# waiwnf/pilotguru

Measured on AMD Instinct MI355X. Metric: frames/sec ORB extract+match, 1080p @ 2000 kp/frame, higher is better.
Workload: dtype u8

## Files before the change

pilotguru_amd/csrc/describe.hip:

```cpp
#include "pgorb_internal.h"

struct PgGauss7 { int k0, k1, k2, k3; };
constexpr PgGauss7 PG_G7 = {18, 34, 49, 55};

#define DH_N 37

struct PgDescTab { uint32_t mom[5 * 64]; uint32_t btab[3 * 64 * 4]; int8_t pat[64 * 4 * 4]; };
constexpr PgDescTab pg_make_desc_tab()
{
    constexpr int umax[16] = {15, 15, 15, 15, 14, 14, 14, 13, 13, 12, 11, 10, 9, 8, 6, 3};
    constexpr int8_t p[256 * 4] = {
#include "orb_pattern31.inc"
    };
    constexpr int K[7] = {PG_G7.k0, PG_G7.k1, PG_G7.k2, PG_G7.k3, PG_G7.k2, PG_G7.k1, PG_G7.k0};
    PgDescTab t = {};
    for (int r = 0; r < 31; r++)
        for (int q = 0; q < 9; q++) {
            const int vy = r - 15, dmax = umax[vy < 0 ? -vy : vy];
            uint32_t wu = 0;
            for (int k = 0; k < 4; k++) {
                const int ux = 4 * (q + 1) + k - 21;
                if ((ux < 0 ? -ux : ux) <= dmax) wu |= (uint32_t)(ux + 16) << (8 * k);
            }
            t.mom[r * 9 + q] = wu;
        }
    for (int cb = 0; cb < 3; cb++)
        for (int l = 0; l < 64; l++)
            for (int j = 0; j < 16; j++) {
                const int k = 16 * (l >> 4) + j, n = 16 * cb + (l & 15), d = k - n;
                const uint32_t v = (d >= 0 && d <= 6 && n < DH_N) ? (uint32_t)K[d] : 0u;
                t.btab[(cb * 64 + l) * 4 + j / 4] |= v << (8 * (j % 4));
            }
    for (int l = 0; l < 64; l++)
        for (int r = 0; r < 4; r++)
            for (int k = 0; k < 4; k++) t.pat[(l * 4 + r) * 4 + k] = p[(64 * r + l) * 4 + k];
    return t;
}
__device__ static const __attribute__((aligned(16))) PgDescTab pg_desc_tab = pg_make_desc_tab();

#define DW_R 21
#define DW_N 43
#define DW_PITCH 48
#define DH_PITCH 40
#define DB_PITCH 40

__device__ __forceinline__ int pg_reflect101(int p, int n)
{
    if (n == 1) return 0;
    while (p < 0 || p >= n) p = (p < 0) ? -p : 2 * (n - 1) - p;
    return p;
}

__device__ __forceinline__ float pg_fast_atan2(float y, float x)
{
    const float scale = (float)(180 / 3.1415926535897932384626433832795);
    const float p1 = 0.9997878412794807f * scale, p3 = -0.3258083974640975f * scale;
    const float p5 = 0.1555786518463281f * scale, p7 = -0.04432655554792128f * scale;
    const float eps = (float)2.2204460492503131e-16;
    const float ax = fabsf(x), ay = fabsf(y);
    float a, c, c2;
    if (ax >= ay) {
        c = __fdiv_rn(ay, __fadd_rn(ax, eps));
        c2 = __fmul_rn(c, c);
        a = __fmul_rn(__fadd_rn(__fmul_rn(__fadd_rn(__fmul_rn(__fadd_rn(__fmul_rn(p7, c2), p5), c2), p3), c2), p1), c);
    } else {
        c = __fdiv_rn(ax, __fadd_rn(ay, eps));
        c2 = __fmul_rn(c, c);
        a = __fsub_rn(90.f, __fmul_rn(__fadd_rn(__fmul_rn(__fadd_rn(__fmul_rn(__fadd_rn(__fmul_rn(p7, c2), p5), c2), p3), c2), p1), c));
    }
    if (x < 0) a = __fsub_rn(180.f, a);
    if (y < 0) a = __fsub_rn(360.f, a);
    return a;
}

__device__ __forceinline__ void pg_sincos_f(float angle, float* s_out, float* c_out)
{
    const double INV_PIO2 = 0.63661977236758138243;
    const double PIO2_HI = 1.57079632673412561417e+00;
    const double PIO2_LO = 6.07710050650619224932e-11;
    const double x = (double)angle;
    const double kd = floor(__dadd_rn(__dmul_rn(x, INV_PIO2), 0.5));
    const double r = __dsub_rn(__dsub_rn(x, __dmul_rn(kd, PIO2_HI)), __dmul_rn(kd, PIO2_LO));
    const double r2 = __dmul_rn(r, r);
    double ps = -1.0 / 355687428096000.0;
    ps = __dadd_rn(__dmul_rn(ps, r2), 1.0 / 1307674368000.0);
    ps = __dsub_rn(__dmul_rn(ps, r2), 1.0 / 6227020800.0);
    ps = __dadd_rn(__dmul_rn(ps, r2), 1.0 / 39916800.0);
    ps = __dsub_rn(__dmul_rn(ps, r2), 1.0 / 362880.0);
    ps = __dadd_rn(__dmul_rn(ps, r2), 1.0 / 5040.0);
    ps = __dsub_rn(__dmul_rn(ps, r2), 1.0 / 120.0);
    ps = __dadd_rn(__dmul_rn(ps, r2), 1.0 / 6.0);
    const double sn = __dsub_rn(r, __dmul_rn(__dmul_rn(r, r2), ps));
    double pc = -1.0 / 6402373705728000.0;
    pc = __dadd_rn(__dmul_rn(pc, r2), 1.0 / 20922789888000.0);
    pc = __dsub_rn(__dmul_rn(pc, r2), 1.0 / 87178291200.0);
    pc = __dadd_rn(__dmul_rn(pc, r2), 1.0 / 479001600.0);
    pc = __dsub_rn(__dmul_rn(pc, r2), 1.0 / 3628800.0);
    pc = __dadd_rn(__dmul_rn(pc, r2), 1.0 / 40320.0);
    pc = __dsub_rn(__dmul_rn(pc, r2), 1.0 / 720.0);
    pc = __dadd_rn(__dmul_rn(pc, r2), 1.0 / 24.0);
    pc = __dsub_rn(__dmul_rn(pc, r2), 0.5);
    const double cs = __dadd_rn(1.0, __dmul_rn(r2, pc));
    const int k = (int)((long long)kd & 3);
    const double s = (k == 0) ? sn : (k == 1) ? cs : (k == 2) ? -sn : -cs;
    const double c = (k == 0) ? cs : (k == 1) ? -sn : (k == 2) ? -cs : sn;
    *s_out = (float)s;
    *c_out = (float)c;
}

__device__ __forceinline__ int pg_wave_sum(int x)
{
    int v = x;
    v += __builtin_amdgcn_update_dpp(0, v, 0x111, 0xf, 0xf, true);
    v += __builtin_amdgcn_update_dpp(0, v, 0x112, 0xf, 0xf, true);
    v += __builtin_amdgcn_update_dpp(0, v, 0x114, 0xf, 0xf, true);
    v += __builtin_amdgcn_update_dpp(0, v, 0x118, 0xf, 0xf, true);
    v += __builtin_amdgcn_update_dpp(0, v, 0x142, 0xa, 0xf, false);
    v += __builtin_amdgcn_update_dpp(0, v, 0x143, 0xc, 0xf, false);
    return __builtin_amdgcn_readlane(v, 63);
}


typedef __attribute__((address_space(1))) const void* pg_gptr_t;
typedef __attribute__((address_space(3))) void* pg_lptr_t;
typedef unsigned short pg_us2 __attribute__((ext_vector_type(2)));
typedef int pg_v4i __attribute__((ext_vector_type(4)));
#define PG_GLOBAL __attribute__((address_space(1)))
typedef PG_GLOBAL const uint8_t* pg_gbytes_t;

__device__ __forceinline__ int pg_blur_at(const uint32_t* hT, int Y, int X, bool tieEven)
{
    constexpr PgGauss7 G = PG_G7;
    const pg_us2 K01 = {(unsigned short)G.k0, (unsigned short)G.k1}, K23 = {(unsigned short)G.k2, (unsigned short)G.k3},
                 K45 = {(unsigned short)G.k2, (unsigned short)G.k1};
    const uint32_t* s = hT + (Y >> 1) * 40 + X;
    const uint32_t p0 = s[0], p1 = s[40], p2 = s[80], p3 = s[120];
    const uint32_t sh = (uint32_t)(Y & 1) << 4;
    const uint32_t a0 = __builtin_amdgcn_alignbit(p1, p0, sh), a1 = __builtin_amdgcn_alignbit(p2, p1, sh),
                   a2 = __builtin_amdgcn_alignbit(p3, p2, sh), last = (p3 >> sh) & 0xFFFFu;
    uint32_t C = __builtin_amdgcn_udot2(__builtin_bit_cast(pg_us2, a0), K01, (uint32_t)G.k0 * last, false);
    C = __builtin_amdgcn_udot2(__builtin_bit_cast(pg_us2, a1), K23, C, false);
    C = __builtin_amdgcn_udot2(__builtin_bit_cast(pg_us2, a2), K45, C, false);
    int v = (int)((C + 32768u) >> 16);
    if (tieEven && (C & 0xFFFFu) == 0x8000u) v &= ~1;
    return min(v, 255);
}

#define PG_WAVE_SYNC() do { __builtin_amdgcn_fence(__ATOMIC_RELEASE, "wavefront"); __builtin_amdgcn_wave_barrier(); \
                            __builtin_amdgcn_fence(__ATOMIC_ACQUIRE, "wavefront"); } while (0)

struct PgDescArgs {
    const int32_t* kpCount;  const PgSelRec* sel;  int64_t selFrame;  pgorb_keypoint* kps;
    uint8_t* desc;  int32_t* n_out;  int32_t nlevels, tieMode, cap_per_frame, slotBeg;
    int32_t slotEnd, writeTotal, slotsPerXcd, pad[5];
};
static_assert(sizeof(PgDescArgs) == 96 && sizeof(PgDescArgs) <= 128, "one s_load_dwordx16 + one s_load_dwordx8");

__global__ __launch_bounds__(64) void k_describe(const PgDescArgs KA)
{
    __shared__ __attribute__((aligned(16))) uint32_t hbuf[22 * DH_PITCH];
    uint8_t* raw = reinterpret_cast<uint8_t*>(hbuf);

    const int lane = threadIdx.x;
    const uint32_t frame = blockIdx.y;
    typedef int32_t pg_i32x16 __attribute__((ext_vector_type(16)));
    typedef uint32_t pg_u32x16 __attribute__((ext_vector_type(16)));
    typedef uint32_t pg_u32x8 __attribute__((ext_vector_type(8)));
    pg_gbytes_t tb = (pg_gbytes_t)(const void*)&pg_desc_tab;
    asm volatile("" : "+s"(tb));
    const uint32_t o4 = 4u * (uint32_t)lane, o16 = 16u * (uint32_t)lane;
    uint32_t mt[5];
#pragma unroll
    for (int it = 0; it < 5; it++) mt[it] = *(const PG_GLOBAL uint32_t*)(tb + (offsetof(PgDescTab, mom) + 256 * it) + o4);
    pg_v4i Bop[3];
#pragma unroll
    for (int cb = 0; cb < 3; cb++) Bop[cb] = *(const PG_GLOBAL pg_v4i*)(tb + (offsetof(PgDescTab, btab) + 1024 * cb) + o16);
    const pg_v4i pat = *(const PG_GLOBAL pg_v4i*)(tb + offsetof(PgDescTab, pat) + o16);
    pg_u32x16 a0;
    pg_u32x8 a1;
    asm volatile("s_load_dwordx16 %0, %2, 0x0\n\ts_load_dwordx8 %1, %2, 0x40\n\ts_waitcnt lgkmcnt(0)"
                 : "=&s"(a0), "=&s"(a1) : "s"(__builtin_amdgcn_kernarg_segment_ptr()) : "memory");
#define PG_A64(T, v, k) reinterpret_cast<T>((uintptr_t)(((uint64_t)(v)[(k) + 1] << 32) | (v)[k]))
    const int32_t* kpCount = PG_A64(const int32_t*, a0, 0);
    const PgSelRec* sel = PG_A64(const PgSelRec*, a0, 2);
    const int64_t selFrame = (int64_t)(((uint64_t)a0[5] << 32) | a0[4]);
    pgorb_keypoint* kps = PG_A64(pgorb_keypoint*, a0, 6);
    uint8_t* desc = PG_A64(uint8_t*, a0, 8);
    int32_t* n_out = PG_A64(int32_t*, a0, 10);
#undef PG_A64
    const int nlevels = (int)a0[12], tieMode = (int)a0[13], cap_per_frame = (int)a0[14], slotBeg = (int)a0[15];
    const int slotEnd = (int)a1[0], writeTotal = (int)a1[1], slotsPerXcd = (int)a1[2];
    const int slot = slotBeg + (int)(blockIdx.x & 7) * slotsPerXcd + (int)(blockIdx.x >> 3);
    const int32_t* kpc = kpCount + frame * PG_MAXL;
    const PgSelRec* recp = sel + ((int64_t)frame * selFrame + slot);
    pg_i32x16 kc;
    pg_u32x8 rec;
    asm volatile("s_load_dwordx16 %0, %2, 0x0\n\ts_load_dwordx8 %1, %3, 0x0\n\ts_waitcnt lgkmcnt(0)" : "=&s"(kc), "=&s"(rec) : "s"(kpc), "s"(recp) : "memory");
    if (slot >= slotEnd) return;
    const int l = (int)(rec[1] >> 16) & 15;
    int total = 0, before = 0;
#pragma unroll
    for (int q = 0; q < PG_MAXL; q++) {
        const int c = kc[q];
        if (q < l) before += c;
        total += c;
    }
    if (writeTotal && blockIdx.x == 0 && lane == 0) n_out[frame] = total;
    if (rec[1] == 0xFFFFFFFFu || l >= nlevels) return;
    const uint32_t cv = rec[0];
    const int idx = before + (int)(rec[1] & 0xFFFFu);
    const int Lpitch = (int)rec[2], Lw = (int)(rec[3] & 0xFFFFu), Lh = (int)(rec[3] >> 16);
    const uint8_t* img = reinterpret_cast<const uint8_t*>((uintptr_t)(((uint64_t)rec[5] << 32) | rec[4]));
    const float Lscale = __uint_as_float(rec[6]), LpatchSize = __uint_as_float(rec[7]);
    const int x = (int)(cv & 0xFFF) + PG_EDGE, y = (int)((cv >> 12) & 0xFFF) + PG_EDGE;
    const int resp = (int)(cv >> 24);
    const int w = Lw, h = Lh;

    const int x0 = x - DW_R, y0 = y - DW_R;
    if (x0 >= 0 && y0 >= 0 && x0 + DW_PITCH <= w && y + DW_R < h) {
        const int lr = lane / 3, lq = lane - 3 * lr;
        const uint8_t* g = img + (int64_t)(y0 + lr) * Lpitch + x0 + 16 * lq;
        if (lr < 21) {
            __builtin_amdgcn_global_load_lds((pg_gptr_t)g, (pg_lptr_t)raw, 16, 0, 0);
            __builtin_amdgcn_global_load_lds((pg_gptr_t)(g + 21 * (int64_t)Lpitch), (pg_lptr_t)(raw + 21 * DW_PITCH), 16, 0, 0);
            if (lr < 1)
                __builtin_amdgcn_global_load_lds((pg_gptr_t)(g + 42 * (int64_t)Lpitch), (pg_lptr_t)(raw + 42 * DW_PITCH), 16, 0, 0);
        }
        __builtin_amdgcn_s_waitcnt(0);
    } else {
        for (int i = lane; i < DW_N * DW_PITCH; i += 64) {
            const int r = i / DW_PITCH, c = i - r * DW_PITCH;
            raw[r * DW_PITCH + c] =
                img[(int64_t)pg_reflect101(y0 + r, h) * Lpitch + pg_reflect101(x0 + c, w)];
        }
    }
    PG_WAVE_SYNC();

    int m10 = 0, m01 = 0;
#pragma unroll
    for (int it = 0; it < 5; it++) {
        const int i = lane + 64 * it;
        if (i >= 31 * 9) break;
        const int r = i / 9, q = i - r * 9;
        const uint32_t val = *reinterpret_cast<const uint32_t*>(raw + (DW_R - 15 + r) * DW_PITCH + 4 * (q + 1));
        const uint32_t wm = ((mt[it] + 0x7F7F7F7Fu) >> 7) & 0x01010101u;
        const int sv = (int)__builtin_amdgcn_udot4(val, wm, 0u, false);
        m10 += (int)__builtin_amdgcn_udot4(val, mt[it], 0u, false) - 16 * sv;
        m01 += (r - 15) * sv;
    }
    m10 = pg_wave_sum(m10);
    m01 = pg_wave_sum(m01);
    const float angle = pg_fast_atan2((float)m01, (float)m10);

    uint32_t* hT = hbuf;
    {
        constexpr int cinit = 128 * (2 * (PG_G7.k0 + PG_G7.k1 + PG_G7.k2) + PG_G7.k3);
        pg_v4i Aop[3];
#pragma unroll
        for (int rb = 0; rb < 3; rb++) {
            Aop[rb] = *reinterpret_cast<const pg_v4i*>(raw + (16 * rb + (lane & 15)) * DW_PITCH + 16 * (lane >> 4));
            Aop[rb].x ^= (int)0x80808080; Aop[rb].y ^= (int)0x80808080; Aop[rb].z ^= (int)0x80808080; Aop[rb].w ^= (int)0x80808080;
        }
        PG_WAVE_SYNC();
#pragma unroll
        for (int rb = 0; rb < 3; rb++) {
            const int pair = 8 * rb + 2 * (lane >> 4);
#pragma unroll
            for (int cb = 0; cb < 3; cb++) {
                const pg_v4i acc = __builtin_amdgcn_mfma_i32_16x16x64_i8(Aop[rb], Bop[cb], pg_v4i{cinit, cinit, cinit, cinit}, 0, 0, 0);
                const int n = 16 * cb + (lane & 15);
                if (n < DH_PITCH) {
                    if (pair < 22) hT[pair * DH_PITCH + n] = (uint32_t)acc.x | ((uint32_t)acc.y << 16);
                    if (pair + 1 < 22) hT[(pair + 1) * DH_PITCH + n] = (uint32_t)acc.z | ((uint32_t)acc.w << 16);
                }
            }
        }
    }
    PG_WAVE_SYNC();
    const int wvec = w & ~3;

    const float factorPI = (float)(3.1415926535897932384626433832795 / 180.f);
    float a, b;
    pg_sincos_f(__fmul_rn(angle, factorPI), &b, &a);
    unsigned long long bits[4];
#pragma unroll
    for (int r = 0; r < 4; r++) {
        const uint32_t pw = (uint32_t)pat[r];
        const float px0 = (float)(int8_t)(pw & 0xFF), py0 = (float)(int8_t)((pw >> 8) & 0xFF);
        const float px1 = (float)(int8_t)((pw >> 16) & 0xFF), py1 = (float)(int8_t)(pw >> 24);
        const int r0 = __float2int_rn(__fadd_rn(__fmul_rn(px0, b), __fmul_rn(py0, a)));
        const int c0 = __float2int_rn(__fsub_rn(__fmul_rn(px0, a), __fmul_rn(py0, b)));
        const int r1 = __float2int_rn(__fadd_rn(__fmul_rn(px1, b), __fmul_rn(py1, a)));
        const int c1 = __float2int_rn(__fsub_rn(__fmul_rn(px1, a), __fmul_rn(py1, b)));
        const int t0 = pg_blur_at(hT, 18 + r0, 18 + c0, tieMode == 0 && x + c0 < wvec);
        const int t1 = pg_blur_at(hT, 18 + r1, 18 + c1, tieMode == 0 && x + c1 < wvec);
        bits[r] = __ballot(t0 < t1);
    }

    if (idx < cap_per_frame && lane == 0) {
        const int64_t o = (int64_t)frame * cap_per_frame + idx;
        unsigned long long* d = reinterpret_cast<unsigned long long*>(desc + o * 32);
        d[0] = bits[0]; d[1] = bits[1]; d[2] = bits[2]; d[3] = bits[3];
        pgorb_keypoint k;
        k.x = (l != 0) ? __fmul_rn((float)x, Lscale) : (float)x;
        k.y = (l != 0) ? __fmul_rn((float)y, Lscale) : (float)y;
        k.size = LpatchSize;
        k.angle = angle;
        k.response = (float)resp;
        k.octave = l;
        k.class_id = -1;
        kps[o] = k;
    }
}

static PgGauss7 pg_gauss7()
{
    float cf[7];
    double sum = 0;
    for (int i = 0; i < 7; i++) {
        const double xx = i - 3.0;
        cf[i] = (float)exp(-0.5 / (2.0 * 2.0) * xx * xx);
        sum += cf[i];
    }
    sum = 1. / sum;
    int K[7];
    for (int i = 0; i < 7; i++) {
        cf[i] = (float)(cf[i] * sum);
        K[i] = (int)lrint((double)(cf[i] * 256.f));
    }
    PgGauss7 g = {K[0], K[1], K[2], K[3]};
    return g;
}

bool pg_launch_describe(const PgPlan& P, int nframes, pgorb_keypoint* d_kps, uint8_t* d_desc,
                        int cap_per_frame, int32_t* d_n, hipStream_t s)
{
    return pg_launch_describe_levels(P, nframes, d_kps, d_desc, cap_per_frame, d_n, 0, P.nlevels, s);
}

bool pg_launch_describe_levels(const PgPlan& P, int nframes, pgorb_keypoint* d_kps, uint8_t* d_desc,
                               int cap_per_frame, int32_t* d_n, int levelBeg, int levelEnd, hipStream_t s)
{
    static const PgGauss7 G = pg_gauss7();
    static const bool tapsOk = G.k0 == PG_G7.k0 && G.k1 == PG_G7.k1 && G.k2 == PG_G7.k2 && G.k3 == PG_G7.k3;
    if (!tapsOk) return false;
    PgDescArgs KA = {};
    KA.kpCount = P.kpCount; KA.sel = reinterpret_cast<const PgSelRec*>(P.sel); KA.selFrame = P.selFrame;
    KA.kps = d_kps; KA.desc = d_desc; KA.n_out = d_n;
    KA.nlevels = P.nlevels; KA.tieMode = P.tieMode; KA.cap_per_frame = cap_per_frame;
    KA.slotBeg = (int)P.lvl[levelBeg].selOff;
    KA.slotEnd = (levelEnd < P.nlevels) ? (int)P.lvl[levelEnd].selOff : P.selTotal;
    KA.writeTotal = levelEnd == P.nlevels ? 1 : 0;
    dim3 grid((KA.slotEnd - KA.slotBeg + 7) & ~7, nframes), block(64);
    KA.slotsPerXcd = (int)(grid.x >> 3);
    hipLaunchKernelGGL(k_describe, grid, block, 0, s, KA);
    return true;
}

__global__ __launch_bounds__(256) void k_sincos_checksum(uint32_t first_bits, uint32_t count, unsigned long long* out)
{
    const uint32_t base = first_bits + blockIdx.x * count;
    unsigned long long acc = 0;
    for (uint32_t i = threadIdx.x; i < count; i += 256) {
        float s, c;
        pg_sincos_f(__uint_as_float(base + i), &s, &c);
        acc += ((unsigned long long)__float_as_uint(s) * 0x9E3779B1ull + __float_as_uint(c)) * (2ull * i + 1ull);
    }
    __shared__ unsigned long long red[256];
    red[threadIdx.x] = acc;
    __syncthreads();
    for (int st = 128; st > 0; st >>= 1) {
        if ((int)threadIdx.x < st) red[threadIdx.x] += red[threadIdx.x + st];
        __syncthreads();
    }
    if (threadIdx.x == 0) out[blockIdx.x] = red[0];
}

extern "C" int pgorb_debug_sincos_checksum(uint32_t first_bits, uint32_t count, int nblocks, unsigned long long* out)
{
    if (!out || nblocks < 1 || count < 1) return PGORB_E_ARG;
    unsigned long long* d = nullptr;
    if (hipMalloc((void**)&d, sizeof(unsigned long long) * (size_t)nblocks) != hipSuccess) return PGORB_E_HIP;
    hipLaunchKernelGGL(k_sincos_checksum, dim3(nblocks), dim3(256), 0, 0, first_bits, count, d);
    const bool ok = hipMemcpy(out, d, sizeof(unsigned long long) * (size_t)nblocks, hipMemcpyDeviceToHost) == hipSuccess;
    (void)hipFree(d);
    return ok ? 0 : PGORB_E_HIP;
}
```

Before: 99640.

## Restructure describe kernel moments, blur buffer layout, and tap address arithmetic

The moment table is reordered so each lane handles one column position across five rows spaced seven apart. This lets the per-row sums chain through udot4 accumulators and removes the per-iteration division and modulo. The blurred-row buffer pitch grows to 48 with 24 row pairs, so all nine MFMA results are stored without bounds checks, and the MFMAs are issued back to back before any stores. Sample coordinates are rounded with a float magic-number add, and the LDS address and tie-break comparison are computed directly from the float bits, replacing float-to-int conversions and integer index math. The larger buffer uses more LDS, and the bit tricks depend on coordinates staying inside a small range.

Result: no change. 100,200, median of 6 (+0.5%).

```diff
diff --git a/pilotguru_amd/csrc/describe.hip b/pilotguru_amd/csrc/describe.hip
--- a/pilotguru_amd/csrc/describe.hip
+++ b/pilotguru_amd/csrc/describe.hip
@@ -22,7 +22,7 @@
                 const int ux = 4 * (q + 1) + k - 21;
                 if ((ux < 0 ? -ux : ux) <= dmax) wu |= (uint32_t)(ux + 16) << (8 * k);
             }
-            t.mom[r * 9 + q] = wu;
+            t.mom[(r / 7) * 64 + (r % 7) * 9 + q] = wu;
         }
     for (int cb = 0; cb < 3; cb++)
         for (int l = 0; l < 64; l++)
@@ -41,7 +41,8 @@
 #define DW_R 21
 #define DW_N 43
 #define DW_PITCH 48
-#define DH_PITCH 40
+#define DH_PITCH 48
+#define DH_PAIRS 24
 #define DB_PITCH 40
 
 __device__ __forceinline__ int pg_reflect101(int p, int n)
@@ -128,14 +129,14 @@
 #define PG_GLOBAL __attribute__((address_space(1)))
 typedef PG_GLOBAL const uint8_t* pg_gbytes_t;
 
-__device__ __forceinline__ int pg_blur_at(const uint32_t* hT, int Y, int X, bool tieEven)
+typedef __attribute__((address_space(3))) const uint32_t* pg_lds_u32p;
+__device__ __forceinline__ int pg_blur_at(pg_lds_u32p s, uint32_t odd, bool tieEven)
 {
     constexpr PgGauss7 G = PG_G7;
     const pg_us2 K01 = {(unsigned short)G.k0, (unsigned short)G.k1}, K23 = {(unsigned short)G.k2, (unsigned short)G.k3},
                  K45 = {(unsigned short)G.k2, (unsigned short)G.k1};
-    const uint32_t* s = hT + (Y >> 1) * 40 + X;
-    const uint32_t p0 = s[0], p1 = s[40], p2 = s[80], p3 = s[120];
-    const uint32_t sh = (uint32_t)(Y & 1) << 4;
+    const uint32_t p0 = s[0], p1 = s[DH_PITCH], p2 = s[2 * DH_PITCH], p3 = s[3 * DH_PITCH];
+    const uint32_t sh = odd << 4;
     const uint32_t a0 = __builtin_amdgcn_alignbit(p1, p0, sh), a1 = __builtin_amdgcn_alignbit(p2, p1, sh),
                    a2 = __builtin_amdgcn_alignbit(p3, p2, sh), last = (p3 >> sh) & 0xFFFFu;
     uint32_t C = __builtin_amdgcn_udot2(__builtin_bit_cast(pg_us2, a0), K01, (uint32_t)G.k0 * last, false);
@@ -158,7 +159,7 @@
 
 __global__ __launch_bounds__(64) void k_describe(const PgDescArgs KA)
 {
-    __shared__ __attribute__((aligned(16))) uint32_t hbuf[22 * DH_PITCH];
+    __shared__ __attribute__((aligned(16))) uint32_t hbuf[DH_PAIRS * DH_PITCH];
     uint8_t* raw = reinterpret_cast<uint8_t*>(hbuf);
 
     const int lane = threadIdx.x;
@@ -236,17 +237,21 @@
     }
     PG_WAVE_SYNC();
 
-    int m10 = 0, m01 = 0;
-#pragma unroll
-    for (int it = 0; it < 5; it++) {
-        const int i = lane + 64 * it;
-        if (i >= 31 * 9) break;
-        const int r = i / 9, q = i - r * 9;
-        const uint32_t val = *reinterpret_cast<const uint32_t*>(raw + (DW_R - 15 + r) * DW_PITCH + 4 * (q + 1));
-        const uint32_t wm = ((mt[it] + 0x7F7F7F7Fu) >> 7) & 0x01010101u;
-        const int sv = (int)__builtin_amdgcn_udot4(val, wm, 0u, false);
-        m10 += (int)__builtin_amdgcn_udot4(val, mt[it], 0u, false) - 16 * sv;
-        m01 += (r - 15) * sv;
+    int m10, m01;
+    {
+        const int r0 = lane / 9, q = lane - 9 * r0;
+        const uint8_t* mrow = raw + (DW_R - 15 + r0) * DW_PITCH + 4 * (q + 1);
+        uint32_t val[5], S[5], mu = 0;
+#pragma unroll
+        for (int it = 0; it < 5; it++) val[it] = *reinterpret_cast<const uint32_t*>(mrow + 7 * it * DW_PITCH);
+#pragma unroll
+        for (int it = 0; it < 5; it++) {
+            const uint32_t wm = ((mt[it] + 0x7F7F7F7Fu) >> 7) & 0x01010101u;
+            S[it] = __builtin_amdgcn_udot4(val[it], wm, it ? S[it - 1] : 0u, false);
+            mu = __builtin_amdgcn_udot4(val[it], mt[it], mu, false);
+        }
+        m10 = (int)mu - 16 * (int)S[4];
+        m01 = __mul24(r0 + 13, (int)S[4]) - __mul24(7, (int)(S[0] + S[1] + S[2] + S[3]));
     }
     m10 = pg_wave_sum(m10);
     m01 = pg_wave_sum(m01);
@@ -262,19 +267,21 @@
             Aop[rb].x ^= (int)0x80808080; Aop[rb].y ^= (int)0x80808080; Aop[rb].z ^= (int)0x80808080; Aop[rb].w ^= (int)0x80808080;
         }
         PG_WAVE_SYNC();
-#pragma unroll
-        for (int rb = 0; rb < 3; rb++) {
-            const int pair = 8 * rb + 2 * (lane >> 4);
+        pg_v4i cini = {cinit, cinit, cinit, cinit};
+        asm volatile("" : "+v"(cini));
+        pg_v4i acc[3][3];
+#pragma unroll
+        for (int rb = 0; rb < 3; rb++)
+#pragma unroll
+            for (int cb = 0; cb < 3; cb++) acc[rb][cb] = __builtin_amdgcn_mfma_i32_16x16x64_i8(Aop[rb], Bop[cb], cini, 0, 0, 0);
+        uint32_t* hs = hT + 2 * (lane >> 4) * DH_PITCH + (lane & 15);
+#pragma unroll
+        for (int rb = 0; rb < 3; rb++)
 #pragma unroll
             for (int cb = 0; cb < 3; cb++) {
-                const pg_v4i acc = __builtin_amdgcn_mfma_i32_16x16x64_i8(Aop[rb], Bop[cb], pg_v4i{cinit, cinit, cinit, cinit}, 0, 0, 0);
-                const int n = 16 * cb + (lane & 15);
-                if (n < DH_PITCH) {
-                    if (pair < 22) hT[pair * DH_PITCH + n] = (uint32_t)acc.x | ((uint32_t)acc.y << 16);
-                    if (pair + 1 < 22) hT[(pair + 1) * DH_PITCH + n] = (uint32_t)acc.z | ((uint32_t)acc.w << 16);
-                }
+                hs[8 * rb * DH_PITCH + 16 * cb] = (uint32_t)acc[rb][cb].x | ((uint32_t)acc[rb][cb].y << 16);
+                hs[(8 * rb + 1) * DH_PITCH + 16 * cb] = (uint32_t)acc[rb][cb].z | ((uint32_t)acc[rb][cb].w << 16);
             }
-        }
     }
     PG_WAVE_SYNC();
     const int wvec = w & ~3;
@@ -283,19 +290,22 @@
     float a, b;
     pg_sincos_f(__fmul_rn(angle, factorPI), &b, &a);
     unsigned long long bits[4];
+    const uint32_t hb = (uint32_t)(uintptr_t)(pg_lptr_t)hT;
+    const float magic = 12582930.0f;
+    const uint32_t hbk = hb - 4u * 0x4B400000u;
+    const int xlim = tieMode == 0 ? wvec - x + 0x4B400012 : (int)0x80000000;
+#define PG_TAP(sr, sc) ({ const uint32_t yb_ = __float_as_uint(__fadd_rn(sr, magic)), xb_ = __float_as_uint(__fadd_rn(sc, magic)); \
+                          pg_blur_at((pg_lds_u32p)(uintptr_t)((((yb_ & 0x3Eu) * (DH_PITCH / 2u) + xb_) << 2) + hbk), yb_ & 1u, (int)xb_ < xlim); })
 #pragma unroll
     for (int r = 0; r < 4; r++) {
         const uint32_t pw = (uint32_t)pat[r];
         const float px0 = (float)(int8_t)(pw & 0xFF), py0 = (float)(int8_t)((pw >> 8) & 0xFF);
         const float px1 = (float)(int8_t)((pw >> 16) & 0xFF), py1 = (float)(int8_t)(pw >> 24);
-        const int r0 = __float2int_rn(__fadd_rn(__fmul_rn(px0, b), __fmul_rn(py0, a)));
-        const int c0 = __float2int_rn(__fsub_rn(__fmul_rn(px0, a), __fmul_rn(py0, b)));
-        const int r1 = __float2int_rn(__fadd_rn(__fmul_rn(px1, b), __fmul_rn(py1, a)));
-        const int c1 = __float2int_rn(__fsub_rn(__fmul_rn(px1, a), __fmul_rn(py1, b)));
-        const int t0 = pg_blur_at(hT, 18 + r0, 18 + c0, tieMode == 0 && x + c0 < wvec);
-        const int t1 = pg_blur_at(hT, 18 + r1, 18 + c1, tieMode == 0 && x + c1 < wvec);
+        const int t0 = PG_TAP(__fadd_rn(__fmul_rn(px0, b), __fmul_rn(py0, a)), __fsub_rn(__fmul_rn(px0, a), __fmul_rn(py0, b)));
+        const int t1 = PG_TAP(__fadd_rn(__fmul_rn(px1, b), __fmul_rn(py1, a)), __fsub_rn(__fmul_rn(px1, a), __fmul_rn(py1, b)));
         bits[r] = __ballot(t0 < t1);
     }
+#undef PG_TAP
 
     if (idx < cap_per_frame && lane == 0) {
         const int64_t o = (int64_t)frame * cap_per_frame + idx;
```
